# lihzha/lap

Hardware: AMD Instinct MI355X
Metric: train-step samples/sec LAP-3B bf16 (higher is better)
Workload: dtype bf16; 1 GPU; LAP-3B (SigLIP So400m/14 + Gemma-2B + Gemma-300M expert) full train step fwd+bwd+AdamW+EMA, 2x224x224 images + 48-token prompt + 50-step action chunk, random-init weights; global_batch=32, per_gpu_batch=32, seq_len=610, parallelism=single

## Files before the change

lap_amd/csrc/attention.hip:

```cpp
#include "common.hpp"
#include "../../include/lap_hip.h"

namespace {

constexpr float NEG_BIG = -1.0e30f;
constexpr float LSE_EMPTY = 1.0e30f;

struct AttnP {
  const bf16* q[2]; bf16* o[2]; const bf16* k[2]; const bf16* v[2];
  const bf16* d_o[2]; bf16* dq[2]; bf16* dk[2]; bf16* dv[2];
  int qlen[2], klen[2];
  int q_rs[2], kv_rs[2], o_rs[2];
  const int32_t* qinfo; const int32_t* kinfo;
  float* lse; float* delta;
  int fuse_delta;
  float scale;
  int B, NH, NKV, stop;
  int hsplit;
  float* part;
  int nsplit;
  float* lpart;
};

template <int HD> struct Cfg {
// ... 400 lines not shown
  }
#pragma unroll
  for (int d = 0; d < C::DF; ++d) {
    const int d0 = d * 16 + 4 * g;
    if (d0 < HD) {
      store4(p.dk[kseg] + koff + d0, acc_dk[d], 1.0f);
      store4(p.dv[kseg] + koff + d0, acc_dv[d], 1.0f);
    }
  }
}

template <int HD>
__global__ __launch_bounds__(256) void attn_dkdv_reduce_kernel(AttnP p) {
  const int Tk = p.klen[0] + p.klen[1];
  const long long n_all = (long long)p.B * Tk * p.NKV * HD;
  const long long i4 = ((long long)blockIdx.x * 256 + threadIdx.x) * 4;
  if (i4 >= n_all) return;
  f32x4 sk = {0.f, 0.f, 0.f, 0.f}, sv = {0.f, 0.f, 0.f, 0.f};
  for (int hgp = 0; hgp < p.hsplit; ++hgp) {
    sk += *reinterpret_cast<const f32x4*>(p.part + (long long)hgp * n_all + i4);
    sv += *reinterpret_cast<const f32x4*>(p.part + ((long long)p.hsplit + hgp) * n_all + i4);
  }
  const int d0 = (int)(i4 % HD);
  long long r = i4 / HD;
  const int hk = (int)(r % p.NKV); r /= p.NKV;
  const int t = (int)(r % Tk);
  const int b = (int)(r / Tk);
  const int seg = t >= p.klen[0];
  const int tt = seg ? t - p.klen[0] : t;
  const long long off = (b * (long long)p.klen[seg] + tt) * p.kv_rs[seg] + hk * HD + d0;
  store4(p.dk[seg] + off, sk, 1.0f);
  store4(p.dv[seg] + off, sv, 1.0f);
}

template <int HD>
__global__ __launch_bounds__(256) void attn_bwd_dq_kernel(AttnP p) {
  using C = Cfg<HD>;
  extern __shared__ __attribute__((aligned(16))) char smem[];
  char* sK = smem;
  char* sV = smem + C::TILE;
  int* sInfo = reinterpret_cast<int*>(smem + 2 * C::TILE);
  const int lane = threadIdx.x & 63, w = threadIdx.x >> 6;
  const int i = lane & 15, g = lane >> 4;
  const BlockId id = decode_block(p.qlen[0], p.qlen[1], p.NH);
  const int b = id.b, h = id.h;
  const int qlen = p.qlen[id.seg];
  const int Tq = p.qlen[0] + p.qlen[1], Tk = p.klen[0] + p.klen[1];
  const int qinfo_off = id.seg ? p.qlen[0] : 0;
  const int myq = id.tile * 64 + w * 16 + i;
  const bool vq = myq < qlen;
  const int hk = h / (p.NH / p.NKV);
  const long long qoff = (b * (long long)qlen + myq) * p.q_rs[id.seg] + h * HD;
  const long long ooff = (b * (long long)qlen + myq) * p.o_rs[id.seg] + h * HD;

  bf16x8 qf[C::KS], dof[C::KS];
  load_row_frags<HD>(p.q[id.seg] + qoff, vq, lane, qf);
  load_row_frags<HD>(p.d_o[id.seg] + ooff, vq, lane, dof);
  const int qi = (p.qinfo && vq) ? p.qinfo[(long long)b * Tq + qinfo_off + myq] : 0x7fffffff;
  const float lse_q = vq ? p.lse[((long long)b * p.NH + h) * Tq + qinfo_off + myq] : LSE_EMPTY;
  const float dl_q = vq ? p.delta[((long long)b * p.NH + h) * Tq + qinfo_off + myq] : 0.f;

  f32x4 acc[C::DF];
#pragma unroll
  for (int d = 0; d < C::DF; ++d) acc[d] = f32x4{0.f, 0.f, 0.f, 0.f};

  for (int ks = 0; ks < 2; ++ks) {
    const int klen = p.klen[ks];
    if (klen == 0) continue;
    const int kinfo_off = ks ? p.klen[0] : 0;
    const long long krs = p.kv_rs[ks];
    const bf16* kb = p.k[ks] + (long long)b * klen * krs + hk * HD;
    const bf16* vb = p.v[ks] + (long long)b * klen * krs + hk * HD;
    for (int kt = 0; kt * 64 < klen; ++kt) {
      __syncthreads();
      const int vr = min(64, klen - kt * 64);
      load_tile<HD>(sK, kb + (long long)kt * 64 * krs, krs, vr);
      load_tile<HD>(sV, vb + (long long)kt * 64 * krs, krs, vr);
      if (p.kinfo) stage_infos(sInfo, p.kinfo + (long long)b * Tk + kinfo_off + kt * 64, vr, false);
      __syncthreads();
      bool all_ok = vr == 64, none = false;
      if (p.kinfo) {
        const int kand = sInfo[64], kor = sInfo[65], kmax = sInfo[66];
        all_ok = all_ok && (((qi >> 24) & kand) != 0) && (kmax <= (qi & 0xffffff));
        none = vq && (((qi >> 24) & kor) == 0);
      }
      if (__all(none || !vq)) continue;
      const bool fast = __all(all_ok || !vq);
      f32x4 s[4], dp[4];
#pragma unroll
      for (int nf = 0; nf < 4; ++nf) { s[nf] = f32x4{0.f, 0.f, 0.f, 0.f}; dp[nf] = f32x4{0.f, 0.f, 0.f, 0.f}; }
#pragma unroll
      for (int kk = 0; kk < C::KS; ++kk)
#pragma unroll
        for (int nf = 0; nf < 4; ++nf) {
          s[nf] = mfma16(frag_kc<HD>(sK, nf * 16, kk, lane), qf[kk], s[nf]);
          dp[nf] = mfma16(frag_kc<HD>(sV, nf * 16, kk, lane), dof[kk], dp[nf]);
        }
#pragma unroll
      for (int nf = 0; nf < 4; ++nf) {
        i32x4 kw = {0, 0, 0, 0};
        if (!fast && p.kinfo) kw = *reinterpret_cast<const i32x4*>(sInfo + nf * 16 + 4 * g);
#pragma unroll
        for (int r = 0; r < 4; ++r) {
          bool a = vq;
          if (!fast) {
            const int key = kt * 64 + nf * 16 + 4 * g + r;
            a = vq && key < klen;
            if (a && p.kinfo) a = mask_ok(qi, kw[r]);
          }
          dp[nf][r] = a ? __expf(s[nf][r] * p.scale - lse_q) * (dp[nf][r] - dl_q) * p.scale : 0.f;
        }
      }
      const bf16x8 d0 = pack8(dp[0], dp[1]), d1 = pack8(dp[2], dp[3]);
#pragma unroll
      for (int d = 0; d < C::DF; ++d) {
        acc[d] = mfma16(frag_tr<HD>(sK, 0, d * 16, lane), d0, acc[d]);
        acc[d] = mfma16(frag_tr<HD>(sK, 32, d * 16, lane), d1, acc[d]);
      }
    }
  }
  if (!vq) return;
#pragma unroll
  for (int d = 0; d < C::DF; ++d) {
    const int d0 = d * 16 + 4 * g;
    if (d0 < HD) store4(p.dq[id.seg] + qoff + d0, acc[d], 1.0f);
  }
}

#include "attention_dma.hpp"

template <typename K>
int set_lds(K kernel, int bytes) {
  if (bytes > 65536) {
    hipError_t e = hipFuncSetAttribute((const void*)kernel, hipFuncAttributeMaxDynamicSharedMemorySize, bytes);
    if (e != hipSuccess) return (int)e;
  }
  return 0;
}

#include "attention_serve.hpp"
#include "serve_chain.hpp"
#include "serve_chain_tp.hpp"

int g_attn_variant = -1;
int attn_variant() { return g_attn_variant; }

constexpr int DMA_MAX_INFO_BYTES = 16384;
bool dma_path_ok(const AttnP& p) {
  const int ntk = (p.klen[0] + 31) / 32 + (p.klen[1] + 31) / 32, ntq = (p.qlen[0] + 31) / 32 + (p.qlen[1] + 31) / 32;
  const int per = (ntk + p.nsplit - 1) / p.nsplit;
  return attn_variant() != 0 && max(ntk, ntq) * 144 <= DMA_MAX_INFO_BYTES && per <= 64 && ntq <= 64 && p.scale > 0.f;
}

template <int HD>
int launch_fwd_dma(const AttnP& p, hipStream_t s) {
  const int nt = (p.qlen[0] + p.qlen[1] + 63) / 64;
  const int ntk = (p.klen[0] + 31) / 32 + (p.klen[1] + 31) / 32;
  const int lds = 4 * DmaCfg<HD>::TILE + ntk * 144;
  auto kern = attn_dma_q_kernel<HD, 0>;
  if (int e = set_lds(kern, lds)) return e;
  hipLaunchKernelGGL(kern, dim3(p.B * p.NH * nt, p.nsplit), dim3(256), lds, s, p);
  LAP_CHECK_LAUNCH();
  return LAP_OK;
}

template <int HD>
int launch_fwd(const AttnP& p, hipStream_t s) {
  if constexpr (HD == 256 || HD == 72) {
    if (dma_path_ok(p)) {
      if (int e = launch_fwd_dma<HD>(p, s)) return e;
      if (p.nsplit > 1) {
        const long long n4 = (long long)p.B * (p.qlen[0] + p.qlen[1]) * p.NH * HD / 4;
        hipLaunchKernelGGL(attn_fwd_combine_kernel<HD>, dim3((unsigned)((n4 + 255) / 256)), dim3(256), 0, s, p);
        LAP_CHECK_LAUNCH();
      }
      return LAP_OK;
    }
  }
  const int nt = (p.qlen[0] + 63) / 64 + (p.qlen[1] + 63) / 64;
  const int lds = 2 * Cfg<HD>::TILE + 1024;
  if (int e = set_lds(attn_fwd_kernel<HD>, lds)) return e;
  hipLaunchKernelGGL(attn_fwd_kernel<HD>, dim3(p.B * p.NH * nt, p.nsplit), dim3(256), lds, s, p);
  LAP_CHECK_LAUNCH();
  if (p.nsplit > 1) {
    const long long n4 = (long long)p.B * (p.qlen[0] + p.qlen[1]) * p.NH * HD / 4;
    hipLaunchKernelGGL(attn_fwd_combine_kernel<HD>, dim3((unsigned)((n4 + 255) / 256)), dim3(256), 0, s, p);
    LAP_CHECK_LAUNCH();
  }
  return LAP_OK;
}
template <int HD>
int launch_bwd(const AttnP& p, hipStream_t s) {
  const int Tq = p.qlen[0] + p.qlen[1];
  const int ntk = (p.klen[0] + 63) / 64 + (p.klen[1] + 63) / 64;
  auto reduce = [&]() -> int {
    if (p.hsplit > 1) {
      const long long n4 = (long long)p.B * (p.klen[0] + p.klen[1]) * p.NKV * HD / 4;
      hipLaunchKernelGGL(attn_dkdv_reduce_kernel<HD>, dim3((unsigned)((n4 + 255) / 256)), dim3(256), 0, s, p);
      LAP_CHECK_LAUNCH();
    }
    return LAP_OK;
  };
  auto delta = [&]() -> int {
    const long long items = (long long)p.B * Tq * p.NH;
    hipLaunchKernelGGL(attn_delta_kernel<HD>, dim3((unsigned)((items + 15) / 16)), dim3(256), 0, s, p);
    LAP_CHECK_LAUNCH();
    return LAP_OK;
  };
  if constexpr (HD == 256 || HD == 72) {
    if (dma_path_ok(p)) {
      AttnP q = p;
      q.fuse_delta = attn_variant() != 2;
      if (!q.fuse_delta) { if (int e = delta()) return e; }
      const int nt = (Tq + 63) / 64;
      const int ntk32 = (p.klen[0] + 31) / 32 + (p.klen[1] + 31) / 32;
      const int lds_q = 4 * DmaCfg<HD>::TILE + ntk32 * 144;
      auto kq = attn_dma_q_kernel<HD, 1>;
      if (int e = set_lds(kq, lds_q)) return e;
      hipLaunchKernelGGL(kq, dim3(p.B * p.NH * nt, 1), dim3(256), lds_q, s, q);
      LAP_CHECK_LAUNCH();
      const int ntq32 = (p.qlen[0] + 31) / 32 + (p.qlen[1] + 31) / 32;
      const int lds_kv = 4 * DmaCfg<HD>::TILE + 1024 + ntq32 * 144;
      auto kkv = attn_dma_kv_kernel<HD>;
      if (int e = set_lds(kkv, lds_kv)) return e;
      hipLaunchKernelGGL(kkv, dim3(p.B * p.NKV * p.hsplit * ntk), dim3(256), lds_kv, s, p);
      LAP_CHECK_LAUNCH();
      return reduce();
    }
  }
  const int lds = 2 * Cfg<HD>::TILE + 1024;
  if (int e = delta()) return e;
  if (int e = set_lds(attn_bwd_dkdv_kernel<HD>, lds)) return e;
  hipLaunchKernelGGL(attn_bwd_dkdv_kernel<HD>, dim3(p.B * p.NKV * p.hsplit * ntk), dim3(256), lds, s, p);
  LAP_CHECK_LAUNCH();
  if (int e = reduce()) return e;
  const int ntq = (p.qlen[0] + 63) / 64 + (p.qlen[1] + 63) / 64;
  if (int e = set_lds(attn_bwd_dq_kernel<HD>, lds)) return e;
  hipLaunchKernelGGL(attn_bwd_dq_kernel<HD>, dim3(p.B * p.NH * ntq), dim3(256), lds, s, p);
  LAP_CHECK_LAUNCH();
  return LAP_OK;
}

bool check_common(int B, int NH, int NKV, int HD, const int* qlen, const int* klen) {
  if (B <= 0 || NH <= 0 || NKV <= 0 || NH % NKV) return false;
  if (HD != 16 && HD != 72 && HD != 256) return false;
  if (qlen[0] < 0 || qlen[1] < 0 || klen[0] < 0 || klen[1] < 0) return false;
  if (qlen[0] + qlen[1] == 0 || klen[0] + klen[1] == 0) return false;
  return true;
}

}

extern "C" int lap_attention_set_variant(int variant) {
  if (variant < -1 || variant > 2) return LAP_ERR_ARG;
  g_attn_variant = variant;
  return LAP_OK;
}

extern "C" int lap_attention_fwd(const lap_attn_fwd_args* a, void* stream) {
  if (!a || !check_common(a->B, a->NH, a->NKV, a->HD, a->q_len, a->k_len)) return LAP_ERR_ARG;
  AttnP p = {};
  for (int s = 0; s < 2; ++s) {
    p.q[s] = (const bf16*)a->q[s]; p.o[s] = (bf16*)a->o[s];
    p.k[s] = (const bf16*)a->k[s]; p.v[s] = (const bf16*)a->v[s];
    p.qlen[s] = a->q_len[s]; p.klen[s] = a->k_len[s];
    p.q_rs[s] = a->q_rs[s] ? a->q_rs[s] : a->NH * a->HD;
    p.o_rs[s] = a->o_rs[s] ? a->o_rs[s] : a->NH * a->HD;
    p.kv_rs[s] = a->kv_rs[s] ? a->kv_rs[s] : a->NKV * a->HD;
    if ((p.q_rs[s] | p.o_rs[s] | p.kv_rs[s]) & 7) return LAP_ERR_ARG;
    if (p.qlen[s] && (!p.q[s] || !p.o[s])) return LAP_ERR_ARG;
    if (p.klen[s] && (!p.k[s] || !p.v[s])) return LAP_ERR_ARG;
  }
  if ((a->qinfo == nullptr) != (a->kinfo == nullptr)) return LAP_ERR_ARG;
  p.qinfo = a->qinfo; p.kinfo = a->kinfo; p.lse = a->lse;
  p.scale = a->scale;
  p.nsplit = 1; p.hsplit = 1;
  if (a->nsplit > 1) {
    const long long Tq = a->q_len[0] + a->q_len[1];
    const long long need = (long long)a->nsplit * a->B * Tq * a->NH * (a->HD + 1);
    if (!a->scratch || a->scratch_floats < need || (a->HD & 3)) return LAP_ERR_ARG;
    p.nsplit = a->nsplit;
    p.part = a->scratch;
    p.lpart = a->scratch + (long long)a->nsplit * a->B * Tq * a->NH * a->HD;
  }
  p.B = a->B; p.NH = a->NH; p.NKV = a->NKV;
  hipStream_t s = (hipStream_t)stream;
  switch (a->HD) {
    case 16: return launch_fwd<16>(p, s);
    case 72: return launch_fwd<72>(p, s);
    case 256: return launch_fwd<256>(p, s);
  }
  return LAP_ERR_ARG;
}

extern "C" int lap_attention_serve_splits(int k_len0, int k_len1, int B, int NH, int q_len1) {
  if (k_len0 < 0 || k_len1 < 0 || k_len0 + k_len1 == 0 || B <= 0 || NH <= 0 || q_len1 <= 0) return 0;
  int cap = serve_run_cap(B, NH, q_len1);
  if (serve_runs(k_len0, k_len1, cap).nruns < 1) cap = (k_len0 + SV_KEYS - 1) / SV_KEYS + (k_len1 + SV_KEYS - 1) / SV_KEYS;
  return cap <= SV_MAX_RUNS ? cap : 0;
}

extern "C" int lap_attention_serve(const lap_attn_fwd_args* a, void* stream) {
  if (!a || !check_common(a->B, a->NH, a->NKV, a->HD, a->q_len, a->k_len)) return LAP_ERR_ARG;
  if (a->HD != 256 || a->q_len[0] != 0 || a->q_len[1] > 64 || a->lse || !a->q[1] || !a->o[1]) return LAP_ERR_ARG;
  AttnP p = {};
  for (int s = 0; s < 2; ++s) {
    p.q[s] = (const bf16*)a->q[s]; p.o[s] = (bf16*)a->o[s];
    p.k[s] = (const bf16*)a->k[s]; p.v[s] = (const bf16*)a->v[s];
    p.qlen[s] = a->q_len[s]; p.klen[s] = a->k_len[s];
    p.q_rs[s] = a->q_rs[s] ? a->q_rs[s] : a->NH * a->HD;
    p.o_rs[s] = a->o_rs[s] ? a->o_rs[s] : a->NH * a->HD;
    p.kv_rs[s] = a->kv_rs[s] ? a->kv_rs[s] : a->NKV * a->HD;
    if ((p.q_rs[s] | p.o_rs[s] | p.kv_rs[s]) & 7) return LAP_ERR_ARG;
    if (p.klen[s] && (!p.k[s] || !p.v[s])) return LAP_ERR_ARG;
    if ((long long)p.klen[s] * p.kv_rs[s] * 2 >= 0x7fffffffLL) return LAP_ERR_ARG;
  }
  if ((a->qinfo == nullptr) != (a->kinfo == nullptr)) return LAP_ERR_ARG;
  p.qinfo = a->qinfo; p.kinfo = a->kinfo; p.scale = a->scale;
  if (!(a->scale > 0.f)) return LAP_ERR_ARG;
  const long long need = (long long)a->nsplit * a->B * a->q_len[1] * a->NH * (a->HD + 1);
  if (a->nsplit < 1 || !a->scratch || a->scratch_floats < need) return LAP_ERR_ARG;
  p.nsplit = a->nsplit; p.hsplit = 1;
  p.part = a->scratch;
  p.lpart = a->scratch + (long long)a->nsplit * a->B * a->q_len[1] * a->NH * a->HD;
  p.B = a->B; p.NH = a->NH; p.NKV = a->NKV;
  return launch_serve(p, (hipStream_t)stream);
}

extern "C" int lap_serve_chain_ok(int B, int S, int D, int H, int NH, int HD, int NKV, int prefix_len) {
  return chain_ok(B, S, D, H, NH, HD, NKV, prefix_len) && chain_device_ok() ? 1 : 0;
}

extern "C" int lap_serve_chain_tp_ok(int B, int S, int D, int H, int NH, int HD, int NKV, int prefix_len) {
  return chain_tp_ok(B, S, D, H, NH, HD, NKV, prefix_len) && chain_device_ok() ? 1 : 0;
}

extern "C" int lap_serve_chain_counter_words(void) { return CH_CTR_WORDS; }

extern "C" int lap_serve_chain_status(const unsigned* counters, int* status) {
  if (!counters || !status) return LAP_ERR_ARG;
  unsigned v = 0;
  if (hipError_t e = hipMemcpy(&v, counters + CH_CTR_STRIDE * CH_CTR_ERR, sizeof(v), hipMemcpyDeviceToHost); e != hipSuccess) return (int)e;
  *status = v != 0;
  return LAP_OK;
}

extern "C" int lap_serve_chain(const lap_serve_chain_args* a, void* stream) {
  if (!a || a->depth < 1 || a->depth > CH_MAX_DEPTH || a->depth > LAP_CHAIN_MAX_DEPTH) return LAP_ERR_ARG;
  if (!chain_ok(a->B, a->S, a->D, a->H, a->NH, a->HD, 1, a->prefix_len)) return LAP_ERR_ARG;
  if (!a->x_in || !a->x_out || !a->mod || !a->rope_table || !a->q || !a->k || !a->v || !a->o || !a->xa || !a->act || !a->attn_scratch ||
      !a->counters || (a->mod_slot_stride & 7) || a->mod_slot_stride < 3 * a->D || (a->packed && !a->xs))
    return LAP_ERR_ARG;
  if ((a->qinfo == nullptr) != (a->kinfo == nullptr)) return LAP_ERR_ARG;
  const int M = a->B * a->S, kv_rs = a->kv_rs ? a->kv_rs : a->HD;
  if ((kv_rs & 7) || (long long)a->prefix_len * kv_rs * 2 >= 0x7fffffffLL) return LAP_ERR_ARG;
  ChainP c = {};
  c.depth = a->depth; c.M = M; c.rps = a->S; c.D = a->D; c.H = a->H; c.NH = a->NH; c.HD = a->HD;
  c.x_in = (const bf16*)a->x_in; c.x_out = (bf16*)a->x_out; c.mod = (const bf16*)a->mod; c.slot_ld = a->mod_slot_stride;
  for (int l = 0; l < a->depth; ++l) {
    if (!a->wqkv[l] || !a->wo[l] || !a->wgu[l] || !a->wd[l] || (a->prefix_len > 0 && (!a->cache_k[l] || !a->cache_v[l]))) return LAP_ERR_ARG;
    if (((uintptr_t)a->wqkv[l] | (uintptr_t)a->wo[l] | (uintptr_t)a->wgu[l] | (uintptr_t)a->wd[l] | (uintptr_t)a->cache_k[l] | (uintptr_t)a->cache_v[l]) & 15)
      return LAP_ERR_ARG;
    c.wqkv[l] = (const bf16*)a->wqkv[l]; c.wo[l] = (const bf16*)a->wo[l]; c.wgu[l] = (const bf16*)a->wgu[l]; c.wd[l] = (const bf16*)a->wd[l];
    c.ck[l] = (const bf16*)a->cache_k[l]; c.cv[l] = (const bf16*)a->cache_v[l];
  }
  c.sr = serve_runs(a->prefix_len, a->S, serve_run_cap(a->B, a->NH, a->S));
  const long long need = (long long)c.sr.nruns * M * a->NH * (a->HD + 1);
  if (a->attn_scratch_floats < need) return LAP_ERR_ARG;
  AttnP& p = c.attn;
  p.qlen[0] = 0; p.qlen[1] = a->S; p.klen[0] = a->prefix_len; p.klen[1] = a->S;
  p.q_rs[0] = p.q_rs[1] = a->NH * a->HD; p.o_rs[0] = p.o_rs[1] = a->NH * a->HD; p.kv_rs[0] = kv_rs; p.kv_rs[1] = a->HD;
  p.qinfo = a->qinfo; p.kinfo = a->kinfo; p.scale = 1.0f;
  p.B = a->B; p.NH = a->NH; p.NKV = 1; p.nsplit = c.sr.nruns; p.hsplit = 1;
  p.part = a->attn_scratch; p.lpart = a->attn_scratch + (long long)c.sr.nruns * M * a->NH * a->HD;
  c.rope = a->rope_table; c.q_scale = a->q_scale; c.eps = a->eps;
  c.q = (bf16*)a->q; c.k = (bf16*)a->k; c.v = (bf16*)a->v; c.o = (bf16*)a->o; c.xa = (bf16*)a->xa; c.act = (bf16*)a->act;
  c.xs = (bf16*)a->xs;
  c.ctrs = a->counters;
  c.clk = (unsigned long long*)a->debug_clock;
  if (a->packed == 2) {
    if (!chain_tp_ok(a->B, a->S, a->D, a->H, a->NH, a->HD, 1, a->prefix_len) || !a->tp_slabs || !a->tp_xs || !a->tp_xn || !a->tp_k || !a->tp_v)
      return LAP_ERR_ARG;
    TpP t;
    t.c = c;
    t.slab_o = a->tp_slabs; t.slab_d = a->tp_slabs + (long long)TP_X * 64 * a->D;
    t.xs8 = (bf16*)a->tp_xs; t.xn8 = (bf16*)a->tp_xn; t.k8 = (bf16*)a->tp_k; t.v8 = (bf16*)a->tp_v;
    return launch_chain_tp(t, (hipStream_t)stream);
  }
  return launch_chain(c, a->packed != 0, (hipStream_t)stream);
}

extern "C" int lap_attention_bwd(const lap_attn_bwd_args* a, void* stream) {
  if (!a || !check_common(a->B, a->NH, a->NKV, a->HD, a->q_len, a->k_len)) return LAP_ERR_ARG;
  if (!a->lse || !a->delta) return LAP_ERR_ARG;
  AttnP p = {};
  for (int s = 0; s < 2; ++s) {
    p.q[s] = (const bf16*)a->q[s]; p.o[s] = (bf16*)a->o[s]; p.d_o[s] = (const bf16*)a->d_o[s];
    p.k[s] = (const bf16*)a->k[s]; p.v[s] = (const bf16*)a->v[s];
    p.dq[s] = (bf16*)a->dq[s]; p.dk[s] = (bf16*)a->dk[s]; p.dv[s] = (bf16*)a->dv[s];
    p.qlen[s] = a->q_len[s]; p.klen[s] = a->k_len[s];
    p.q_rs[s] = a->q_rs[s] ? a->q_rs[s] : a->NH * a->HD;
    p.o_rs[s] = a->o_rs[s] ? a->o_rs[s] : a->NH * a->HD;
    p.kv_rs[s] = a->kv_rs[s] ? a->kv_rs[s] : a->NKV * a->HD;
    if ((p.q_rs[s] | p.o_rs[s] | p.kv_rs[s]) & 7) return LAP_ERR_ARG;
    if (p.qlen[s] && (!p.q[s] || !p.o[s] || !p.d_o[s] || !p.dq[s])) return LAP_ERR_ARG;
    if (p.klen[s] && (!p.k[s] || !p.v[s] || !p.dk[s] || !p.dv[s])) return LAP_ERR_ARG;
  }
// ... 24 lines not shown
```

lap_amd/csrc/attention_dma.hpp:

```cpp

constexpr int T32_TILE = 32 * 512;

template <int HD> struct DmaCfg;
template <> struct DmaCfg<256> {
  static constexpr int KS = 8, DF = 16, PITCH = 512, REAL_CHUNKS = 32, TILE = 32 * 512, PIECES = 4, KREGS = 4, VREGS = 8, BLOCKS = 2, KV_BLOCKS = 1;
  __device__ static __forceinline__ int swz(int row) { return (row & 7) << 1; }
};
template <> struct DmaCfg<72> {
  static constexpr int KS = 3, DF = 5, PITCH = 256, REAL_CHUNKS = 9, TILE = 32 * 256, PIECES = 2, KREGS = 3, VREGS = 5, BLOCKS = 4, KV_BLOCKS = 3;
  __device__ static __forceinline__ int swz(int row) { return ((row & 7) << 1) | ((row >> 3) & 1); }
};
template <int HD>
__device__ __forceinline__ void dma_lane(int w, int j, int lane, int& row, int& col) {
  using C = DmaCfg<HD>;
  constexpr int CPR = C::PITCH / 16;
  const int piece = w * C::PIECES + j;
  row = piece * (1024 / C::PITCH) + lane / CPR;
  const int c = (lane % CPR) ^ C::swz(row);
  col = c < C::REAL_CHUNKS ? c * 16 : -1;
}
template <int HD>
__device__ __forceinline__ void dma_frag_bases(const char* smem, int lane, const char* (&kbase)[DmaCfg<HD>::KREGS], unsigned (&vbase)[DmaCfg<HD>::VREGS]) {
  using C = DmaCfg<HD>;
  const int i = lane & 15, g = lane >> 4;
// ... 225 lines not shown
          d0[r] = a0 ? __builtin_amdgcn_exp2f(s0[r] * c2 - lse2) * (d0[r] - dl_q) * p.scale : 0.f;
          d1[r] = a1 ? __builtin_amdgcn_exp2f(s1[r] * c2 - lse2) * (d1[r] - dl_q) * p.scale : 0.f;
        }
      }
      const bf16x8 pb = pack8(d0, d1);
      if constexpr (HD == 256) {
      bf16x4 vr[2][8];
#define LAP_ISSUE_K(GRP, R)                                                               \
  _Pragma("unroll") for (int j = 0; j < 4; ++j) {                                         \
    R[2 * j] = ds_read_tr_raw<KOFF + ((GRP) >> 1) * 256>(va[((GRP) & 1) * 4 + j]);        \
    R[2 * j + 1] = ds_read_tr_raw<KOFF + ((GRP) >> 1) * 256 + 16 * 512>(va[((GRP) & 1) * 4 + j]); \
  }
#define LAP_DQ(GRP, R)                                                                    \
  _Pragma("unroll") for (int j = 0; j < 4; ++j)                                           \
    acc_o[(GRP) * 4 + j] = mfma16(join8(R[2 * j], R[2 * j + 1]), pb, acc_o[(GRP) * 4 + j]);
      LAP_ISSUE_K(0, vr[0])
      LAP_ISSUE_K(1, vr[1]) lds_wait8<8>(vr[0]); LAP_DQ(0, vr[0])
      LAP_ISSUE_K(2, vr[0]) lds_wait8<8>(vr[1]); LAP_DQ(1, vr[1])
      LAP_ISSUE_K(3, vr[1]) lds_wait8<8>(vr[0]); LAP_DQ(2, vr[0])
      lds_wait8<0>(vr[1]); LAP_DQ(3, vr[1])
#undef LAP_ISSUE_K
#undef LAP_DQ
      } else {
        bf16x4 vr[2 * DF];
        tr_burst<HD, KOFF>(va, vr);
#pragma unroll
        for (int d = 0; d < DF; ++d) acc_o[d] = mfma16(join8(vr[2 * d], vr[2 * d + 1]), pb, acc_o[d]);
      }
      return;
    }
    f32x4 s0 = {0.f, 0.f, 0.f, 0.f}, s1 = {0.f, 0.f, 0.f, 0.f};
#pragma unroll
    for (int kk = 0; kk < KS; ++kk) {
      const bf16x8 k0 = *reinterpret_cast<const bf16x8*>(kp[kreg<HD>(kk)] + KOFF + kimm<HD>(kk));
      const bf16x8 k1 = *reinterpret_cast<const bf16x8*>(kp[kreg<HD>(kk)] + KOFF + 16 * PITCH + kimm<HD>(kk));
      s0 = mfma16(k0, qf[kk], s0);
      s1 = mfma16(k1, qf[kk], s1);
    }
    i32x4 kw0 = {0, 0, 0, 0}, kw1 = {0, 0, 0, 0};
    bool ok0[4], ok1[4];
    float mx;
    if (fast) {
      mx = fmaxf(fmaxf(fmaxf(s0[0], s0[1]), fmaxf(s0[2], s0[3])), fmaxf(fmaxf(s1[0], s1[1]), fmaxf(s1[2], s1[3])));
    } else {
      kw0 = *reinterpret_cast<const i32x4*>(sWords + gt * 32 + 4 * g);
      kw1 = *reinterpret_cast<const i32x4*>(sWords + gt * 32 + 16 + 4 * g);
      mx = NEG_BIG;
#pragma unroll
      for (int r = 0; r < 4; ++r) {
        ok0[r] = (qcls & (kw0[r] >> 24)) != 0 && (kw0[r] & 0xffffff) <= qidx;
        ok1[r] = (qcls & (kw1[r] >> 24)) != 0 && (kw1[r] & 0xffffff) <= qidx;
        if (ok0[r]) mx = fmaxf(mx, s0[r]);
        if (ok1[r]) mx = fmaxf(mx, s1[r]);
      }
    }
    const float m_new = fmaxf(m, max_over_groups(mx) * c2);
    if (__any(m_new > m + 8.0f)) {
      const float alpha = __builtin_amdgcn_exp2f(m - m_new);
      l *= alpha;
#pragma unroll
      for (int d = 0; d < DF; ++d) acc_o[d] *= alpha;
      m = m_new;
    }
    if (fast) {
#pragma unroll
      for (int r = 0; r < 4; ++r) {
        s0[r] = __builtin_amdgcn_exp2f(s0[r] * c2 - m);
        s1[r] = __builtin_amdgcn_exp2f(s1[r] * c2 - m);
      }
    } else {
#pragma unroll
      for (int r = 0; r < 4; ++r) {
        s0[r] = ok0[r] ? __builtin_amdgcn_exp2f(s0[r] * c2 - m) : 0.f;
        s1[r] = ok1[r] ? __builtin_amdgcn_exp2f(s1[r] * c2 - m) : 0.f;
      }
    }
    l += ((s0[0] + s0[1]) + (s0[2] + s0[3])) + ((s1[0] + s1[1]) + (s1[2] + s1[3]));
    const bf16x8 pb = pack8(s0, s1);

    if constexpr (HD == 256) {
    bf16x4 vr[2][8];
#define LAP_ISSUE_V(GRP, R)                                                               \
  _Pragma("unroll") for (int j = 0; j < 4; ++j) {                                         \
    R[2 * j] = ds_read_tr_raw<VOFF + ((GRP) >> 1) * 256>(va[((GRP) & 1) * 4 + j]);        \
    R[2 * j + 1] = ds_read_tr_raw<VOFF + ((GRP) >> 1) * 256 + 16 * 512>(va[((GRP) & 1) * 4 + j]); \
  }
#define LAP_PV(GRP, R)                                                                    \
  _Pragma("unroll") for (int j = 0; j < 4; ++j)                                           \
    acc_o[(GRP) * 4 + j] = mfma16(join8(R[2 * j], R[2 * j + 1]), pb, acc_o[(GRP) * 4 + j]);
    LAP_ISSUE_V(0, vr[0])
    LAP_ISSUE_V(1, vr[1]) lds_wait8<8>(vr[0]); LAP_PV(0, vr[0])
    LAP_ISSUE_V(2, vr[0]) lds_wait8<8>(vr[1]); LAP_PV(1, vr[1])
    LAP_ISSUE_V(3, vr[1]) lds_wait8<8>(vr[0]); LAP_PV(2, vr[0])
    lds_wait8<0>(vr[1]); LAP_PV(3, vr[1])
#undef LAP_ISSUE_V
#undef LAP_PV
    } else {
      bf16x4 vr[2 * DF];
      tr_burst<HD, VOFF>(va, vr);
#pragma unroll
      for (int d = 0; d < DF; ++d) acc_o[d] = mfma16(join8(vr[2 * d], vr[2 * d + 1]), pb, acc_o[d]);
    }
  };

  if (gt0 < gt1) issue(0);
  stage_infos();
  __syncthreads();
  {
    const int t = gt0 + lane;
    i32x4 sm = {0, 0, 0, 0};
    if (t < gt1) sm = *reinterpret_cast<const i32x4*>(sSum + t * 4);
    bool f = sm[3] == 32;
    int qor = 0;
#pragma unroll
    for (int r = 0; r < 16; ++r) {
      const int c = __builtin_amdgcn_readlane(qcls, r), x = __builtin_amdgcn_readlane(qidx, r);
      qor |= c;
      f = f && (c & sm[0]) != 0 && sm[2] <= x;
    }
    skipmask = __ballot((qor & sm[1]) == 0);
    fastmask = __ballot(f);
  }
  for (int gt = gt0; gt < gt1; gt += 2) {
    step(IC<0>{}, gt);
    if (gt + 1 < gt1) step(IC<1>{}, gt + 1);
  }

  if (MODE == 1) {
    if (!vq) return;
    bf16* dqrow = p.dq[qsg] + (b * (long long)p.qlen[qsg] + qloc) * p.q_rs[qsg] + h * HD;
#pragma unroll
    for (int d = 0; d < DF; ++d)
      if (d * 16 + 4 * g < HD) store4(dqrow + d * 16 + 4 * g, acc_o[d], 1.0f);
    return;
  }
  l = sum_over_groups(l);
  if (!vq) return;
  const float inv = l > 0.f ? 1.0f / l : 0.f;
  const float lse = (m + __builtin_amdgcn_logf(l)) * LN2;
  if (p.nsplit > 1) {
    const long long row = ((long long)blockIdx.y * p.B + b) * Tq + myq;
    float* op = p.part + (row * p.NH + h) * HD;
#pragma unroll
    for (int d = 0; d < DF; ++d)
      if (d * 16 + 4 * g < HD) *reinterpret_cast<f32x4*>(op + d * 16 + 4 * g) = acc_o[d] * inv;
    if (g == 0) p.lpart[(((long long)blockIdx.y * p.B + b) * p.NH + h) * Tq + myq] = l > 0.f ? lse : NEG_BIG;
    return;
  }
  bf16* orow = p.o[qsg] + (b * (long long)p.qlen[qsg] + qloc) * p.o_rs[qsg] + h * HD;
#pragma unroll
  for (int d = 0; d < DF; ++d)
    if (d * 16 + 4 * g < HD) store4(orow + d * 16 + 4 * g, acc_o[d], inv);
  if (p.lse && g == 0) p.lse[((long long)b * p.NH + h) * Tq + myq] = l > 0.f ? lse : LSE_EMPTY;
}

template <int HD>
__global__ __launch_bounds__(256, DmaCfg<HD>::KV_BLOCKS) void attn_dma_kv_kernel(AttnP p) {
  using C = DmaCfg<HD>;
  constexpr int KS = C::KS, DF = C::DF, TILE = C::TILE, PITCH = C::PITCH;
  extern __shared__ __attribute__((aligned(16))) char smem[];
  const int lane = threadIdx.x & 63, w = __builtin_amdgcn_readfirstlane(threadIdx.x >> 6);
  const int i = lane & 15, g = lane >> 4;
  const BlockId id = decode_block(p.klen[0], p.klen[1], p.NKV * p.hsplit);
  const int b = id.b, hk = id.h / p.hsplit, hg = id.h % p.hsplit, kseg = id.seg;
  const int klen = p.klen[kseg];
  const int Tq = p.qlen[0] + p.qlen[1], Tk = p.klen[0] + p.klen[1];
  const int mykey = id.tile * 64 + w * 16 + i;
  const bool vk = mykey < klen;
  const long long koff = (b * (long long)klen + mykey) * p.kv_rs[kseg] + hk * HD;
  const int nq0 = (p.qlen[0] + 31) >> 5, nq1 = (p.stop && kseg == 0) ? 0 : (p.qlen[1] + 31) >> 5, ntq = nq0 + nq1;
  float* sLD = reinterpret_cast<float*>(smem + 4 * TILE);
  int* sWords = reinterpret_cast<int*>(smem + 4 * TILE + 1024);
  int* sSum = sWords + ntq * 32;

  bf16x8 kf[KS], vf[KS];
  load_row_frags<HD>(p.k[kseg] + koff, vk, lane, kf);
  load_row_frags<HD>(p.v[kseg] + koff, vk, lane, vf);
  const int ki = !vk ? 0 : (p.kinfo ? p.kinfo[(long long)b * Tk + (kseg ? p.klen[0] : 0) + mykey] : 0x7f000000);
  const int kcls = ki >> 24, kidx = ki & 0xffffff;

  for (int base = w; base < ntq; base += 32) {
    int v[8], valid[8];
#pragma unroll
    for (int u = 0; u < 8; ++u) {
      const int t = base + 4 * u;
      const int sg = t >= nq0, tl = sg ? t - nq0 : t;
      valid[u] = t < ntq ? min(32, p.qlen[sg] - tl * 32) : 0;
      v[u] = 0;
      if (lane < valid[u]) v[u] = p.qinfo ? p.qinfo[(long long)b * Tq + (sg ? p.qlen[0] : 0) + tl * 32 + lane] : 0x7fffffff;
    }
#pragma unroll
    for (int u = 0; u < 8; ++u) {
      const int t = base + 4 * u;
      if (t < ntq) put_infos32(sWords + t * 32, sSum + t * 4, v[u], valid[u], lane, true);
    }
  }

  const int hpk = p.NH / p.NKV, hpg = hpk / p.hsplit;
  const int h_first = hk * hpk + hg * hpg;
  const int items = hpg * ntq;
  int cur_h = h_first, cur_t = 0;
  int dma_row[C::PIECES], dma_col[C::PIECES];
#pragma unroll
  for (int j = 0; j < C::PIECES; ++j) dma_lane<HD>(w, j, lane, dma_row[j], dma_col[j]);
  auto issue = [&](int stage) {
    const int sg = cur_t >= nq0, tl = sg ? cur_t - nq0 : cur_t;
    const int qlen = p.qlen[sg], qrs = p.q_rs[sg], ors = p.o_rs[sg];
    const auto rsQ = __builtin_amdgcn_make_buffer_rsrc((void*)(p.q[sg] + (long long)b * qlen * qrs + cur_h * HD), 0, seg_records(qlen, qrs, HD), 0x00020000);
    const auto rsD = __builtin_amdgcn_make_buffer_rsrc((void*)(p.d_o[sg] + (long long)b * qlen * ors + cur_h * HD), 0, seg_records(qlen, ors, HD), 0x00020000);
    char* base = smem + stage * 2 * TILE;
#pragma unroll
    for (int j = 0; j < C::PIECES; ++j) {
      char* dst = base + (w * C::PIECES + j) * 1024;
      const unsigned oq = dma_col[j] < 0 ? DMA_OOB : (unsigned)((tl * 32 + dma_row[j]) * qrs * 2 + dma_col[j]);
      const unsigned od = dma_col[j] < 0 ? DMA_OOB : (unsigned)((tl * 32 + dma_row[j]) * ors * 2 + dma_col[j]);
      __builtin_amdgcn_raw_ptr_buffer_load_lds(rsQ, (LDS_PTR(void))dst, 16, oq, 0, 0, 0);
      __builtin_amdgcn_raw_ptr_buffer_load_lds(rsD, (LDS_PTR(void))(dst + TILE), 16, od, 0, 0, 0);
    }
    if (w == 0) {
      const long long roff = ((long long)b * p.NH + cur_h) * Tq + (sg ? p.qlen[0] : 0);
      const auto rsL = __builtin_amdgcn_make_buffer_rsrc((void*)(p.lse + roff), 0, qlen * 4, 0x00020000);
      const auto rsX = __builtin_amdgcn_make_buffer_rsrc((void*)(p.delta + roff), 0, qlen * 4, 0x00020000);
      const unsigned off = lane < 32 ? (unsigned)((tl * 32 + lane) * 4) : DMA_OOB;
      float* dst = sLD + stage * 128;
      __builtin_amdgcn_raw_ptr_buffer_load_lds(rsL, (LDS_PTR(void))dst, 4, off, 0, 0, 0);
      __builtin_amdgcn_raw_ptr_buffer_load_lds(rsX, (LDS_PTR(void))(dst + 64), 4, off, 0, 0, 0);
    }
    if (++cur_t == ntq) { cur_t = 0; ++cur_h; }
  };

  const char* kp[C::KREGS];
  unsigned va[C::VREGS];
  dma_frag_bases<HD>(smem, lane, kp, va);
  unsigned ka[C::KREGS];
#pragma unroll
  for (int c = 0; c < C::KREGS; ++c) ka[c] = lds_addr_of(kp[c]);

  const float c2 = p.scale * LOG2E;
  f32x4 acc_dk[DF], acc_dv[DF];
#pragma unroll
  for (int d = 0; d < DF; ++d) { acc_dk[d] = f32x4{0.f, 0.f, 0.f, 0.f}; acc_dv[d] = f32x4{0.f, 0.f, 0.f, 0.f}; }

  unsigned long long skipmask = 0, fastmask = 0;
  auto step = [&](auto STC, int qt) {
    constexpr int ST = decltype(STC)::value;
    constexpr int QOFF = ST * 2 * TILE, DOFF = QOFF + TILE;
    wait_vm0();
    __syncthreads();
    if (cur_h < h_first + hpg) issue(ST ^ 1);
    if ((skipmask >> qt) & 1) return;
    const bool fast = (fastmask >> qt) & 1;

    f32x4 s0 = {0.f, 0.f, 0.f, 0.f}, s1 = {0.f, 0.f, 0.f, 0.f}, d0 = {0.f, 0.f, 0.f, 0.f}, d1 = {0.f, 0.f, 0.f, 0.f};
    const float* ld = sLD + ST * 128;
    f32x4 l0 = *reinterpret_cast<const f32x4*>(ld + 4 * g) * LOG2E, l1 = *reinterpret_cast<const f32x4*>(ld + 16 + 4 * g) * LOG2E;
    f32x4 x0 = *reinterpret_cast<const f32x4*>(ld + 64 + 4 * g), x1 = *reinterpret_cast<const f32x4*>(ld + 80 + 4 * g);
    if constexpr (HD == 256) { lds_tie(l0); lds_tie(l1); lds_tie(x0); lds_tie(x1); }
    if constexpr (HD == 256) {
      bf16x8 fr[32];
#define LAP_RQ(KK) \
      fr[4 * KK] = ds_read_b128_raw<QOFF + kimm<HD>(KK)>(ka[kreg<HD>(KK)]); \
      fr[4 * KK + 1] = ds_read_b128_raw<QOFF + 16 * PITCH + kimm<HD>(KK)>(ka[kreg<HD>(KK)]); \
      fr[4 * KK + 2] = ds_read_b128_raw<DOFF + kimm<HD>(KK)>(ka[kreg<HD>(KK)]); \
      fr[4 * KK + 3] = ds_read_b128_raw<DOFF + 16 * PITCH + kimm<HD>(KK)>(ka[kreg<HD>(KK)]);
#define LAP_SQ(KK, LEFT) \
      lds_wait4x<LEFT>(fr[4 * KK], fr[4 * KK + 1], fr[4 * KK + 2], fr[4 * KK + 3]); \
      s0 = mfma16(fr[4 * KK], kf[KK], s0); s1 = mfma16(fr[4 * KK + 1], kf[KK], s1); \
      d0 = mfma16(fr[4 * KK + 2], vf[KK], d0); d1 = mfma16(fr[4 * KK + 3], vf[KK], d1);
      LAP_RQ(0) LAP_RQ(1) LAP_RQ(2)
      LAP_SQ(0, 8) LAP_RQ(3)
      LAP_SQ(1, 8) LAP_RQ(4)
      LAP_SQ(2, 8) LAP_RQ(5)
      LAP_SQ(3, 8) LAP_RQ(6)
      LAP_SQ(4, 8) LAP_RQ(7)
      LAP_SQ(5, 8) LAP_SQ(6, 4) LAP_SQ(7, 0)
#undef LAP_RQ
#undef LAP_SQ
    } else {
#pragma unroll
    for (int kk = 0; kk < KS; ++kk) {
      const bf16x8 q0 = *reinterpret_cast<const bf16x8*>(kp[kreg<HD>(kk)] + QOFF + kimm<HD>(kk));
      const bf16x8 q1 = *reinterpret_cast<const bf16x8*>(kp[kreg<HD>(kk)] + QOFF + 16 * PITCH + kimm<HD>(kk));
      const bf16x8 o0 = *reinterpret_cast<const bf16x8*>(kp[kreg<HD>(kk)] + DOFF + kimm<HD>(kk));
      const bf16x8 o1 = *reinterpret_cast<const bf16x8*>(kp[kreg<HD>(kk)] + DOFF + 16 * PITCH + kimm<HD>(kk));
      s0 = mfma16(q0, kf[kk], s0);
      s1 = mfma16(q1, kf[kk], s1);
      d0 = mfma16(o0, vf[kk], d0);
      d1 = mfma16(o1, vf[kk], d1);
    }
    }
    if (fast) {
#pragma unroll
      for (int r = 0; r < 4; ++r) {
        s0[r] = __builtin_amdgcn_exp2f(s0[r] * c2 - l0[r]);
        s1[r] = __builtin_amdgcn_exp2f(s1[r] * c2 - l1[r]);
        d0[r] = s0[r] * (d0[r] - x0[r]) * p.scale;
        d1[r] = s1[r] * (d1[r] - x1[r]) * p.scale;
      }
    } else {
      const i32x4 qw0 = *reinterpret_cast<const i32x4*>(sWords + qt * 32 + 4 * g);
      const i32x4 qw1 = *reinterpret_cast<const i32x4*>(sWords + qt * 32 + 16 + 4 * g);
#pragma unroll
      for (int r = 0; r < 4; ++r) {
        const bool a0 = ((qw0[r] >> 24) & kcls) != 0 && kidx <= (qw0[r] & 0xffffff);
        const bool a1 = ((qw1[r] >> 24) & kcls) != 0 && kidx <= (qw1[r] & 0xffffff);
        s0[r] = a0 ? __builtin_amdgcn_exp2f(s0[r] * c2 - l0[r]) : 0.f;
// ... 86 lines not shown
```

Measured before the change: 123.8 samples/s.

## Add two-pass full-row forward attention kernel for short SigLIP sequences

Adds a forward attention kernel for head dim 72 that, when the key length fits in eight 32-row tiles and there is no masking info or split, first computes all QK scores into registers to find the exact row max, then does a single exp/PV pass. This replaces the online-softmax rescaling and the per-tile info table of the generic DMA kernel, and keeps the K and V loads double-buffered in LDS. It costs more registers to hold the full score row. It only covers the vision tower's bidirectional attention, which is a small part of the full training step.

```diff
diff --git a/lap_amd/csrc/attention.hip b/lap_amd/csrc/attention.hip
--- a/lap_amd/csrc/attention.hip
+++ b/lap_amd/csrc/attention.hip
@@ -576,10 +576,22 @@
   return attn_variant() != 0 && max(ntk, ntq) * 144 <= DMA_MAX_INFO_BYTES && per <= 64 && ntq <= 64 && p.scale > 0.f;
 }
 
+bool fullrow_ok(const AttnP& p, int HD) {
+  const int ntk = (p.klen[0] + 31) / 32 + (p.klen[1] + 31) / 32;
+  return HD == 72 && !p.qinfo && !p.kinfo && ntk <= FULLROW_TILES && p.nsplit == 1 && attn_variant() != 3;
+}
+
 template <int HD>
 int launch_fwd_dma(const AttnP& p, hipStream_t s) {
   const int nt = (p.qlen[0] + p.qlen[1] + 63) / 64;
   const int ntk = (p.klen[0] + 31) / 32 + (p.klen[1] + 31) / 32;
+  if constexpr (HD == 72) {
+    if (fullrow_ok(p, HD)) {
+      hipLaunchKernelGGL(attn_dma_fullrow_kernel<HD>, dim3(p.B * p.NH * nt), dim3(256), 4 * DmaCfg<HD>::TILE, s, p);
+      LAP_CHECK_LAUNCH();
+      return LAP_OK;
+    }
+  }
   const int lds = 4 * DmaCfg<HD>::TILE + ntk * 144;
   auto kern = attn_dma_q_kernel<HD, 0>;
   if (int e = set_lds(kern, lds)) return e;
@@ -590,6 +602,7 @@
 
 template <int HD>
 int launch_fwd(const AttnP& p, hipStream_t s) {
+  if (attn_variant() == 4 && !(dma_path_ok(p) && fullrow_ok(p, HD))) return LAP_ERR_ARG;
   if constexpr (HD == 256 || HD == 72) {
     if (dma_path_ok(p)) {
       if (int e = launch_fwd_dma<HD>(p, s)) return e;
@@ -676,7 +689,7 @@
 }
 
 extern "C" int lap_attention_set_variant(int variant) {
-  if (variant < -1 || variant > 2) return LAP_ERR_ARG;
+  if (variant < -1 || variant > 4) return LAP_ERR_ARG;
   g_attn_variant = variant;
   return LAP_OK;
 }
diff --git a/lap_amd/csrc/attention_dma.hpp b/lap_amd/csrc/attention_dma.hpp
--- a/lap_amd/csrc/attention_dma.hpp
+++ b/lap_amd/csrc/attention_dma.hpp
@@ -401,6 +401,155 @@
   for (int d = 0; d < DF; ++d)
     if (d * 16 + 4 * g < HD) store4(orow + d * 16 + 4 * g, acc_o[d], inv);
   if (p.lse && g == 0) p.lse[((long long)b * p.NH + h) * Tq + myq] = l > 0.f ? lse : LSE_EMPTY;
+}
+
+constexpr int FULLROW_TILES = 8;
+template <int HD>
+__global__ __launch_bounds__(256, DmaCfg<HD>::BLOCKS) void attn_dma_fullrow_kernel(AttnP p) {
+  using C = DmaCfg<HD>;
+  constexpr int KS = C::KS, DF = C::DF, BQ = 64, TILE = C::TILE, PITCH = C::PITCH, NT = FULLROW_TILES;
+  static_assert(NT == 8 && C::VREGS == DF, "four pair steps per sweep; one address register per d-fragment");
+  extern __shared__ __attribute__((aligned(16))) char smem[];
+  const int lane = threadIdx.x & 63, w = __builtin_amdgcn_readfirstlane(threadIdx.x >> 6);
+  const int i = lane & 15, g = lane >> 4;
+  const int Tq = p.qlen[0] + p.qlen[1];
+  const int ntq = (Tq + BQ - 1) / BQ;
+  const int bid = xcd_remap(blockIdx.x, gridDim.x);
+  const int qtile = bid % ntq, h = (bid / ntq) % p.NH, b = bid / (ntq * p.NH);
+  const int hk = h / (p.NH / p.NKV);
+  const int nt0 = (p.klen[0] + 31) >> 5, nt1 = (p.klen[1] + 31) >> 5, ntk = nt0 + nt1;
+  const int np = (ntk + 1) >> 1, npe = (np + 1) & ~1;
+
+  const int myq = qtile * BQ + w * 16 + i;
+  const bool vq = myq < Tq;
+  const int qsg = myq >= p.qlen[0], qloc = myq - (qsg ? p.qlen[0] : 0);
+  bf16x8 qf[KS];
+  load_row_frags<HD>(p.q[qsg] + (b * (long long)p.qlen[qsg] + qloc) * p.q_rs[qsg] + h * HD, vq, lane, qf);
+
+  const int rowbytes0 = p.kv_rs[0] * 2, rowbytes1 = p.kv_rs[1] * 2;
+  const long long kvoff0 = (long long)b * p.klen[0] * p.kv_rs[0] + hk * HD, kvoff1 = (long long)b * p.klen[1] * p.kv_rs[1] + hk * HD;
+  const auto rsK0 = __builtin_amdgcn_make_buffer_rsrc((void*)(p.k[0] + kvoff0), 0, seg_records(p.klen[0], p.kv_rs[0], HD), 0x00020000);
+  const auto rsV0 = __builtin_amdgcn_make_buffer_rsrc((void*)(p.v[0] + kvoff0), 0, seg_records(p.klen[0], p.kv_rs[0], HD), 0x00020000);
+  const auto rsK1 = __builtin_amdgcn_make_buffer_rsrc((void*)(p.k[1] + kvoff1), 0, seg_records(p.klen[1], p.kv_rs[1], HD), 0x00020000);
+  const auto rsV1 = __builtin_amdgcn_make_buffer_rsrc((void*)(p.v[1] + kvoff1), 0, seg_records(p.klen[1], p.kv_rs[1], HD), 0x00020000);
+  int dma_row[C::PIECES], dma_col[C::PIECES];
+#pragma unroll
+  for (int j = 0; j < C::PIECES; ++j) dma_lane<HD>(w, j, lane, dma_row[j], dma_col[j]);
+  using Rsrc = decltype(rsK0);
+  auto issue_pair = [&](const Rsrc& rs0, const Rsrc& rs1, int stage, int j) {
+#pragma unroll
+    for (int u = 0; u < 2; ++u) {
+      const int t = 2 * j + u;
+      if (t >= ntk) break;
+      const int sg = t >= nt0, tl = sg ? t - nt0 : t;
+      const int rb = sg ? rowbytes1 : rowbytes0;
+      char* base = smem + (2 * stage + u) * TILE;
+#pragma unroll
+      for (int jj = 0; jj < C::PIECES; ++jj) {
+        const unsigned off = dma_col[jj] < 0 ? DMA_OOB : (unsigned)((tl * 32 + dma_row[jj]) * rb + dma_col[jj]);
+        char* dst = base + (w * C::PIECES + jj) * 1024;
+        if (sg == 0) __builtin_amdgcn_raw_ptr_buffer_load_lds(rs0, (LDS_PTR(void))dst, 16, off, 0, 0, 0);
+        else __builtin_amdgcn_raw_ptr_buffer_load_lds(rs1, (LDS_PTR(void))dst, 16, off, 0, 0, 0);
+      }
+    }
+  };
+
+  const char* kp[C::KREGS];
+  unsigned va[C::VREGS];
+  dma_frag_bases<HD>(smem, lane, kp, va);
+
+  const float c2 = p.scale * LOG2E;
+  f32x4 S[2 * NT];
+  float mx = NEG_BIG;
+
+  auto ktile = [&](auto TC, auto SLOT) {
+    constexpr int T = decltype(TC)::value, KOFF = decltype(SLOT)::value * TILE;
+    if (T >= ntk) return;
+    f32x4 s0 = {0.f, 0.f, 0.f, 0.f}, s1 = {0.f, 0.f, 0.f, 0.f};
+#pragma unroll
+    for (int kk = 0; kk < KS; ++kk) {
+      const bf16x8 k0 = *reinterpret_cast<const bf16x8*>(kp[kreg<HD>(kk)] + KOFF + kimm<HD>(kk));
+      const bf16x8 k1 = *reinterpret_cast<const bf16x8*>(kp[kreg<HD>(kk)] + KOFF + 16 * PITCH + kimm<HD>(kk));
+      s0 = mfma16(k0, qf[kk], s0);
+      s1 = mfma16(k1, qf[kk], s1);
+    }
+    const int valid = T >= nt0 ? p.klen[1] - (T - nt0) * 32 : p.klen[0] - T * 32;
+    if (valid < 32) {
+#pragma unroll
+      for (int r = 0; r < 4; ++r) {
+        if (4 * g + r >= valid) s0[r] = NEG_BIG;
+        if (16 + 4 * g + r >= valid) s1[r] = NEG_BIG;
+      }
+    }
+    mx = fmaxf(mx, fmaxf(fmaxf(fmaxf(s0[0], s0[1]), fmaxf(s0[2], s0[3])), fmaxf(fmaxf(s1[0], s1[1]), fmaxf(s1[2], s1[3]))));
+    S[2 * T] = s0;
+    S[2 * T + 1] = s1;
+  };
+  auto kstep = [&](auto JC) {
+    constexpr int J = decltype(JC)::value, ST = J & 1;
+    wait_vm0();
+    __syncthreads();
+    if (J + 1 < npe) issue_pair(rsK0, rsK1, ST ^ 1, J + 1);
+    else issue_pair(rsV0, rsV1, 0, 0);
+    ktile(IC<2 * J>{}, IC<2 * ST>{});
+    ktile(IC<2 * J + 1>{}, IC<2 * ST + 1>{});
+  };
+
+  float m = 0.f, l = 0.f;
+  f32x4 acc_o[DF];
+#pragma unroll
+  for (int d = 0; d < DF; ++d) acc_o[d] = f32x4{0.f, 0.f, 0.f, 0.f};
+  auto vtile = [&](auto TC, auto SLOT) {
+    constexpr int T = decltype(TC)::value, VOFF = decltype(SLOT)::value * TILE;
+    if (T >= ntk) return;
+    bf16x4 vr[2 * DF];
+#pragma unroll
+    for (int d = 0; d < DF; ++d) {
+      vr[2 * d] = ds_read_tr_raw<VOFF>(va[d]);
+      vr[2 * d + 1] = ds_read_tr_raw<VOFF + 16 * PITCH>(va[d]);
+    }
+    f32x4 s0 = S[2 * T], s1 = S[2 * T + 1];
+#pragma unroll
+    for (int r = 0; r < 4; ++r) {
+      s0[r] = __builtin_amdgcn_exp2f(s0[r] * c2 - m);
+      s1[r] = __builtin_amdgcn_exp2f(s1[r] * c2 - m);
+    }
+    l += ((s0[0] + s0[1]) + (s0[2] + s0[3])) + ((s1[0] + s1[1]) + (s1[2] + s1[3]));
+    const bf16x8 pb = pack8(s0, s1);
+    lds_wait_all();
+#pragma unroll
+    for (int d = 0; d < 2 * DF; ++d) lds_tie(vr[d]);
+#pragma unroll
+    for (int d = 0; d < DF; ++d) acc_o[d] = mfma16(join8(vr[2 * d], vr[2 * d + 1]), pb, acc_o[d]);
+  };
+  auto vstep = [&](auto JC) {
+    constexpr int J = decltype(JC)::value, ST = J & 1;
+    wait_vm0();
+    __syncthreads();
+    if (J + 1 < np) issue_pair(rsV0, rsV1, ST ^ 1, J + 1);
+    vtile(IC<2 * J>{}, IC<2 * ST>{});
+    vtile(IC<2 * J + 1>{}, IC<2 * ST + 1>{});
+  };
+
+  issue_pair(rsK0, rsK1, 0, 0);
+  kstep(IC<0>{});
+  kstep(IC<1>{});
+  if (npe > 2) { kstep(IC<2>{}); kstep(IC<3>{}); }
+  m = max_over_groups(mx) * c2;
+  vstep(IC<0>{});
+  if (np > 1) vstep(IC<1>{});
+  if (np > 2) vstep(IC<2>{});
+  if (np > 3) vstep(IC<3>{});
+
+  l = sum_over_groups(l);
+  if (!vq) return;
+  const float inv = 1.0f / l;
+  const float lse = (m + __builtin_amdgcn_logf(l)) * LN2;
+  bf16* orow = p.o[qsg] + (b * (long long)p.qlen[qsg] + qloc) * p.o_rs[qsg] + h * HD;
+#pragma unroll
+  for (int d = 0; d < DF; ++d)
+    if (d * 16 + 4 * g < HD) store4(orow + d * 16 + 4 * g, acc_o[d], inv);
+  if (p.lse && g == 0) p.lse[((long long)b * p.NH + h) * Tq + myq] = lse;
 }
 
 template <int HD>
```

Measured after the change: 123.6 samples/s. Within noise of the previous version (-0.2%).
